# NeuralRevenant/semantic-query-engine

Measured on AMD Instinct MI355X. Metric: k-NN queries/sec (brute-force cosine top-10, 1024-d, 10M vectors), higher is better.
Workload: dtype i8; 1 GPU; flat cosine top-10, N=10000000 x 1024 fp32 (int8 collect scan (per-row-scaled int8 copy, sample-derived thresholds) + fp32 re-score of the candidates, exactness certified per query, bf16 collect pass for uncertified queries), batch=1024 queries/step, index row-sharded over 1 GPU(s); rows=10000000, dim=1024, batch=1024, k=10, parallelism=shard1, scan_mode=int8

## Files before the change

### semantic_query_engine_amd/csrc/exact.hip

```cpp
#include "kernels.h"

namespace sqe {

namespace {

struct RescoreArgs {
    const float* master;
    const float* qn;
    int K, B, k;
    const int* unc_ids;
    const int* unc_count;
    const float* collect_thr;
    uint64_t* keys;
    const int* key_cnt;
    float* cos_out;
    int64_t* id_out;
    int64_t id_base;
};

__global__ __launch_bounds__(256) void collect_rescore_kernel(RescoreArgs p) {
    __shared__ int hist[256];
    __shared__ int scratch[4];
    __shared__ uint64_t top[MAX_KP];
    const int ci = blockIdx.x;
// ... 90 lines not shown
            thr_out[ci] = collect_thr[q];
        }
        __syncthreads();
        if (tid == 0) {
            int t = 0;
            for (int w = 0; w < 16; ++w) t += wave_tot[w];
            base += t;
        }
        __syncthreads();
    }
    const int count = base;
    if (tid == 0) *unc_count = count;
    for (int i = count + tid; i < thr_cap; i += 1024) thr_out[i] = INFINITY;
    __syncthreads();
    const int vec_per_row = row_bytes / 16;
    for (int64_t e = tid; e < (int64_t)count * vec_per_row; e += 1024) {
        const int ci = (int)(e / vec_per_row), v = (int)(e - (int64_t)ci * vec_per_row);
        const uint4* src = reinterpret_cast<const uint4*>(reinterpret_cast<const char*>(qb) + (size_t)unc_ids[ci] * pitch_bytes);
        uint4* dst = reinterpret_cast<uint4*>(reinterpret_cast<char*>(qb_out) + (size_t)ci * pitch_bytes);
        dst[v] = src[v];
    }
}

}

int launch_compact_uncertified(const float* collect_thr, int B, const bf16_t* qb, int pitch_bytes, int row_bytes, int* unc_ids,
                               float* thr_out, int thr_cap, bf16_t* qb_out, int* unc_count, hipStream_t stream) {
    if (B <= 0) return SQE_OK;
    hipLaunchKernelGGL(compact_uncertified_kernel, dim3(1), dim3(1024), 0, stream, collect_thr, B, qb, pitch_bytes, row_bytes,
                       unc_ids, thr_out, thr_cap, qb_out, unc_count);
    SQE_HIP(hipGetLastError());
    return SQE_OK;
}

int launch_collect_rescore(const ExactArgs& a, hipStream_t stream) {
    if (a.B <= 0) return SQE_OK;
    if (a.K % 4 != 0) return fail(SQE_ERR_INVALID, "collect rescore: dim must be a multiple of 4");
    RescoreArgs p;
    p.master = a.master; p.qn = a.qn; p.K = a.K; p.B = a.B; p.k = a.k; p.collect_thr = a.collect_thr;
    p.unc_ids = a.unc_ids; p.unc_count = a.unc_count;
    p.keys = a.keys; p.key_cnt = a.key_cnt; p.cos_out = a.cos_out; p.id_out = a.id_out; p.id_base = a.id_base;
    hipLaunchKernelGGL(collect_rescore_kernel, dim3(a.B), dim3(256), 0, stream, p);
    SQE_HIP(hipGetLastError());
    return SQE_OK;
}

// ... 2 lines not shown
```

### semantic_query_engine_amd/csrc/internal.h

```cpp
#pragma once

#include <atomic>
#include <mutex>
#include <string>
#include <vector>

#include "kernels.h"

namespace sqe {

struct DevBuf {
    void* p = nullptr;
    size_t bytes = 0;
    DevBuf() = default;
    DevBuf(const DevBuf&) = delete;
    DevBuf& operator=(const DevBuf&) = delete;
    ~DevBuf() { release(); }
    void release() {
        if (p) (void)hipFree(p);
        p = nullptr;
        bytes = 0;
    }
    int ensure(size_t need) {
        if (need <= bytes) return SQE_OK;
// ... 144 lines not shown
    sqe::DevBuf dbg;
    sqe::DevBuf resid_max;
    sqe::DevBuf q_resid;
    sqe::DevBuf unc;
    sqe::DevBuf fb_keys, fb_cnt;
    sqe::DevBuf unc_ids, thr_c, qb_c;
    sqe::DevBuf stage_in, stage_out;
    int certify = 1;
    sqe::DevBuf i8db;
    sqe::DevBuf i8sxi;
    sqe::DevBuf i8resid_max;
    int64_t i8_cap_tiles = 0, i8_tile_stride = 0;
    int64_t i8_rows = 0;
    sqe::DevBuf q8t;
    sqe::DevBuf q8, q8sqi, q8resid, i8thr_int, i8thr_eff, i8cos_s, i8ids_s, i8stats, i8samp;
    int64_t i8_min_rows = 1000000;
    int i8_sample_step = 100;
    int i8_sample_m = 20;
    float i8_dx = 0.f;
    bool i8_dx_stale = true;
    bool i8_oom_logged = false;
    int i8_sample_int8 = 1;
    double i8_max_resid = 0.02;
    sqe::DevBuf i8ovf, i8ovf_cnt;
    double i8_anchor_margin = 0.25;
    int i8_key_budget = 6144;
    sqe_i8_launch_t i8_launch{};
    int last_B = 0;
    bool last_i8 = false;
    sqe::IvfState* ivf = nullptr;
    bool internal = false;
    sqe::GroupIndex* group = nullptr;
    std::atomic<int64_t> next_id{0};
    bool has_map = false;
    sqe::DevBuf idmap;
    sqe::FilterState* filter = nullptr;
    int64_t filter_gather_rows = 1 << 20;
    sqe::RangeState* range = nullptr;
    int64_t range_key_budget = 1 << 25;
    bool has_keys = false;
    sqe::DevBuf keys;
    sqe::CollapseState* collapse = nullptr;
    int collapse_depth = 0;
};

struct sqe_cache {
// ... 37 lines not shown
    bool locked;
    OpScope(sqe_ctx* c, OpOrder& ord, bool host_call, bool lock = true) : o(ord), locked(lock) {
        (void)hipSetDevice(c->device);
        if (locked) o.mu.lock();
        s = (host_call && !c->foreign.load()) ? o.own : c->stream.load();
        if (o.armed && o.last != s) (void)hipStreamWaitEvent(s, o.ev, 0);
    }
    ~OpScope() {
        (void)hipEventRecord(o.ev, s);
        o.last = s;
        o.armed = true;
        if (locked) o.mu.unlock();
    }
    OpScope(const OpScope&) = delete;
    OpScope& operator=(const OpScope&) = delete;
};

int index_create_impl(sqe_ctx* ctx, int dim, int kind, int nlist, bool internal, sqe_index** out);
int index_grow(sqe_index* idx, int64_t need_rows, hipStream_t s);
int index_add_impl(sqe_index* idx, const float* x_dev, int64_t n, int64_t x_stride, bool restore, hipStream_t s);
int index_update_impl(sqe_index* idx, const int64_t* rows_dev, const float* x_dev, int64_t n, hipStream_t s);
int index_search_impl(sqe_index* idx, const float* q_dev, int B, int k, int nprobe, float* cos_out_dev, int64_t* id_out_dev,
                      hipStream_t s, int pass_index = 0);

int ivf_create(sqe_index* base, IvfState** out);
void ivf_destroy(IvfState* st);
int ivf_rows_added(sqe_index* base, IvfState* st, hipStream_t s);
int ivf_rows_updated(sqe_index* base, IvfState* st, const int64_t* rows_dev, int64_t n, hipStream_t s);
int ivf_train(sqe_index* base, IvfState* st, const float* x_dev, int64_t n, int iters, uint64_t seed, hipStream_t s);
int ivf_search(sqe_index* base, IvfState* st, const float* q_dev, int B, int k, int nprobe, float* cos_out, int64_t* id_out,
               hipStream_t s);
int ivf_export(sqe_index* base, IvfState* st, float* centroids_host, int32_t* assign_host, hipStream_t s);
void ivf_invalidate(IvfState* st);
sqe_index* ivf_coarse(IvfState* st);
bool ivf_trained(IvfState* st);
int ivf_restore(sqe_index* base, IvfState* st, const float* centroids_dev, const int32_t* assign_dev, int64_t n, hipStream_t s);
void ivf_assignments(IvfState* st, int** assign, int64_t* n_assigned);
void ivf_rows_deleted(IvfState* st, int64_t n_assigned);

int64_t search_id_base(const sqe_index* idx);
int index_translate_ids(sqe_index* idx, int64_t* id_dev, int64_t count, hipStream_t s);
int index_resolve_ids(sqe_index* idx, const int64_t* ids_host, int64_t m, std::vector<int64_t>& pos, hipStream_t s, const char* what);
int index_delete_positions(sqe_index* idx, const std::vector<int64_t>& pos_sorted, hipStream_t s);
int index_ids_host(sqe_index* idx, std::vector<int64_t>& out, hipStream_t s);
int index_set_ids(sqe_index* idx, const int64_t* ids_host, int64_t next_id, hipStream_t s);
int launch_idmap_iota(int64_t* map, int64_t first_pos, int64_t first_id, int64_t n, hipStream_t s);
// ... 60 lines not shown
```

### semantic_query_engine_amd/csrc/search.hip

```cpp
#include <stdio.h>
#include <stdlib.h>
#include <string.h>

#include <algorithm>
#include <tuple>
#include <utility>

#include "internal.h"

namespace sqe {

__global__ void add_count_kernel(int* acc, const int* v) { *acc += *v; }

namespace {

int auto_kp(const sqe_index* idx, int k) {
    if (idx->rescore_k > 0) return std::min(MAX_KP, std::max(idx->rescore_k, k));
    if (idx->certify) return k <= 32 ? 64 : k <= 128 ? 128 : k;
    return std::min(MAX_KP, std::max(32, 4 * k));
}

struct Pass {
    sqe_index* idx;
    hipStream_t s;
    int64_t n_rows;
    int B, k, kp;
    ScanPlan plan;
    float* cos_out;
    int64_t* id_out;
    int pass_index;
    bool certify;
    int* unc_count;
    float* collect_thr;
    int step8, m8;
};

bool i8_stamps_wanted() {
    static const bool want_stamps = [] { const char* e = knob_env("SQE_I8_STAMPS"); return e && e[0] == '1'; }();
    return want_stamps;
}

bool scan_counters_wanted() {
    static const bool want = [] { const char* e = knob_env("SQE_DBG"); return e && (atoi(e) & 32); }();
    return want;
}

int arm_dbg(sqe_index* idx, hipStream_t s, unsigned long long** slot) {
    SQE_TRY(idx->dbg.ensure(8192));
    SQE_HIP(hipMemsetAsync(idx->dbg.p, 0, 8192, s));
    *slot = idx->dbg.as<unsigned long long>();
    return SQE_OK;
}

int report_i8_stamps(sqe_index* idx, hipStream_t s) {
    unsigned long long h[256];
    SQE_HIP(hipMemcpyAsync(h, idx->dbg.p, sizeof(h), hipMemcpyDeviceToHost, s));
    SQE_HIP(hipStreamSynchronize(s));
    int wall_khz = 0;
// ... 109 lines not shown
        idx->i8_tile_stride = stride;
    }
    if (!idx->i8resid_max.p) {
        SQE_TRY(idx->i8resid_max.ensure(16));
        SQE_HIP(hipMemsetAsync(idx->i8resid_max.p, 0, 16, s));
    }
    if (idx->i8_rows < n_rows) {
        StageTimer t(idx->ctx->prof, s, ST_ADD);
        SQE_TRY(launch_quantize_rows_i8(idx->master, nullptr, idx->i8_rows, n_rows - idx->i8_rows, n_rows, K, idx->i8db.as<int8_t>(), stride,
                                        idx->i8sxi.as<uint32_t>(), idx->i8resid_max.as<uint32_t>(), s));
        idx->i8_rows = n_rows;
        idx->i8_dx_stale = true;
    }
    if (idx->i8_dx_stale) {
        uint32_t bits = 0;
        SQE_HIP(hipMemcpyAsync(&bits, idx->i8resid_max.p, 4, hipMemcpyDeviceToHost, s));
        SQE_HIP(hipStreamSynchronize(s));
        memcpy(&idx->i8_dx, &bits, 4);
        idx->i8_dx_stale = false;
    }
    return SQE_OK;
}

int prepare_pass(Pass& p, const float* q_dev) {
    sqe_index* idx = p.idx;
    sqe_ctx* c = idx->ctx;
    const ScanPlan& plan = p.plan;
    hipStream_t s = p.s;
    const int K = idx->dim, B = p.B;
    SQE_TRY(idx->qn.ensure((size_t)B * K * 4));
    SQE_TRY(idx->qb.ensure((size_t)plan.b_pad * idx->pitch));
    SQE_TRY(idx->cand.ensure((size_t)plan.n_chunks * plan.b_pad * CAND_CAP * 8));
    SQE_TRY(idx->cand_cnt.ensure((size_t)plan.n_chunks * plan.b_pad * 4));
    const size_t gmax_bytes = (size_t)plan.b_pad * plan.ngroups * GMAX_COLS * 4;
    SQE_TRY(idx->gmax.ensure(gmax_bytes));
    static const bool no_collect = [] { const char* e = knob_env("SQE_NO_COLLECT"); return e && atoi(e) != 0; }();
    p.certify = idx->certify && p.n_rows > 0 && !no_collect;
    SQE_TRY(idx->q_resid.ensure((size_t)B * 4));
    if (p.certify) {
        SQE_TRY(idx->unc.ensure(16 + (size_t)plan.b_pad * 4));
        SQE_TRY(idx->fb_keys.ensure((size_t)B * EXACT_CAP * 8));
        SQE_TRY(idx->fb_cnt.ensure((size_t)B * 4));
        SQE_TRY(idx->unc_ids.ensure((size_t)B * 4));
        SQE_TRY(idx->thr_c.ensure((size_t)(plan.b_pad + 256) * 4));
        if ((size_t)(plan.b_pad + 256) * idx->pitch > idx->qb_c.bytes) {
            SQE_TRY(idx->qb_c.ensure((size_t)(plan.b_pad + 256) * idx->pitch));
            SQE_HIP(hipMemsetAsync(idx->qb_c.p, 0, idx->qb_c.bytes, s));
        }
    }
    {
        StageTimer t(c->prof, s, ST_PREP);
        if (plan.b_pad > B)
            SQE_HIP(hipMemsetAsync(idx->qb.as<char>() + (size_t)B * idx->pitch, 0, (size_t)(plan.b_pad - B) * idx->pitch, s));
        SQE_TRY(launch_normalize_rows(q_dev, B, K, K, idx->qn.as<float>(), idx->qb.as<bf16_t>(), idx->pitch / 2,
                                      idx->q_resid.as<float>(), nullptr, s));
        if (p.certify) {
            SQE_HIP(hipMemsetAsync(idx->unc.p, 0, 16, s));
            SQE_HIP(hipMemsetAsync(idx->fb_cnt.p, 0, (size_t)B * 4, s));
        }
        SQE_HIP(hipMemsetAsync(idx->gmax.p, 0, gmax_bytes, s));
    }
    p.unc_count = p.certify ? idx->unc.as<int>() : nullptr;
    p.collect_thr = p.certify ? reinterpret_cast<float*>(idx->unc.as<int>() + 4) : nullptr;
    return SQE_OK;
}

std::pair<int, int> sample_plan(int64_t n_rows, int step8, int m8) {
    const int64_t tiles = (n_rows + SCAN_BM - 1) / SCAN_BM;
    const int min_tiles = 2 * GMAX_COLS;
    if (tiles / step8 < min_tiles && tiles / min_tiles >= 1 && tiles / min_tiles < step8) {
        const int step_e = (int)std::max<int64_t>(std::max(1, (step8 * m8 + 63) / 64), tiles / min_tiles);
        const int m_e = std::min(64, std::max(m8, (step8 * m8 + step_e - 1) / step_e));
        step8 = step_e;
        m8 = m_e;
    }
    return {step8, m8};
}

int admit_i8(const Pass& p, bool* use) {
    sqe_index* idx = p.idx;
    const int K = idx->dim;
    *use = idx->scan_mode == SQE_SCAN_INT8_RESCORE && p.certify && K >= 256 && K % 128 == 0 && p.k <= p.m8 &&
           p.n_rows >= idx->i8_min_rows && p.n_rows >= (int64_t)p.step8 * SCAN_BM * 4;
    if (!*use) return SQE_OK;
    const int rc8 = ensure_i8_copy(idx, p.s);
    if (rc8 == SQE_ERR_OOM) {
// ... 2 lines not shown
        idx->scan_mode = SQE_SCAN_BF16_RESCORE;
        *use = false;
    } else {
        SQE_TRY(rc8);
        *use = idx->i8_dx <= (float)idx->i8_max_resid;
    }
    return SQE_OK;
}

ScanArgs bf16_scan_args(const Pass& p, const bf16_t* q) {
    sqe_index* idx = p.idx;
    ScanArgs a;
    a.db = idx->scan; a.q = q; a.n_rows = p.n_rows; a.K = idx->dim; a.B = p.B;
    a.db_pitch = idx->pitch; a.q_pitch = idx->pitch;
    a.cand = idx->cand.as<uint64_t>(); a.cand_cnt = idx->cand_cnt.as<int>(); a.gmax = idx->gmax.as<uint32_t>();
    return a;
}

int run_collect_fallback(const Pass& p) {
    sqe_index* idx = p.idx;
    sqe_ctx* c = idx->ctx;
    hipStream_t s = p.s;
    const int K = idx->dim, B = p.B;
    {
        StageTimer t(c->prof, s, ST_SELECT);
        SQE_TRY(launch_compact_uncertified(p.collect_thr, B, idx->qb.as<bf16_t>(), idx->pitch, K * 2, idx->unc_ids.as<int>(),
                                           idx->thr_c.as<float>(), p.plan.b_pad + 256, idx->qb_c.as<bf16_t>(), p.unc_count, s));
    }
    {
        StageTimer t(c->prof, s, ST_COLLECT);
        ScanArgs a = bf16_scan_args(p, idx->qb_c.as<bf16_t>());
        a.collect_thr = idx->thr_c.as<float>(); a.collect_keys = idx->fb_keys.as<uint64_t>(); a.collect_cnt = idx->fb_cnt.as<int>();
        a.unc_count = p.unc_count;
        const int bounds[5] = {0, 64, 256, 512, 1 << 30};
        for (int r = 0; r < 4 && bounds[r] < B; ++r) {
            const int hi = std::min(bounds[r + 1], B);
            const ScanPlan cp = make_scan_plan(p.n_rows, hi, p.kp, c->cu_count);
            a.collect_lo = bounds[r] + 1;
            a.collect_hi = r == 3 ? (1 << 30) : bounds[r + 1];
            SQE_TRY(launch_scan_collect(cp, a, s));
        }
    }
    {
        StageTimer t(c->prof, s, ST_SELECT);
        ExactArgs e;
        e.master = idx->master; e.qn = idx->qn.as<float>(); e.K = K; e.B = B; e.k = p.k;
        e.collect_thr = p.collect_thr; e.keys = idx->fb_keys.as<uint64_t>(); e.key_cnt = idx->fb_cnt.as<int>();
// ... 68 lines not shown
        ia.qblocks = plan.qblocks; ia.bn = plan.bn; ia.cand = idx->cand.as<uint64_t>(); ia.cand_cnt = idx->cand_cnt.as<int>();
        ia.ovf = idx->i8ovf.as<uint64_t>(); ia.ovf_cnt = idx->i8ovf_cnt.as<int>();
        if (i8_stamps_wanted()) SQE_TRY(arm_dbg(idx, s, &ia.stamps));
        static const int deep_max = [] { const char* e = knob_env("SQE_I8_DEEP_MAX"); return e ? atoi(e) : 1; }();
        if (plan.bn == 256 && plan.qblocks <= deep_max) SQE_TRY(launch_scan_i8_deep(ia, s));
        else SQE_TRY(launch_scan_i8(ia, s));
        if (i8_stamps_wanted()) SQE_TRY(report_i8_stamps(idx, s));
    }
    {
        StageTimer t(c->prof, s, ST_SELECT);
        I8SelectArgs sa;
        sa.cand = idx->cand.as<uint64_t>(); sa.cand_cnt = idx->cand_cnt.as<int>(); sa.n_chunks = plan.n_chunks; sa.b_pad = plan.b_pad;
        sa.master = idx->master; sa.qn = idx->qn.as<float>(); sa.K = K; sa.B = B; sa.k = p.k;
        sa.scan16 = idx->scan; sa.pitch16 = idx->pitch;
        sa.sxi = idx->i8sxi.as<uint32_t>(); sa.sqi = idx->q8sqi.as<uint32_t>();
        sa.q_resid8 = idx->q8resid.as<float>(); sa.db_resid8_max = idx->i8resid_max.as<uint32_t>();
        sa.q_resid16 = idx->q_resid.as<float>(); sa.db_resid16_max = idx->resid_max.as<uint32_t>();
        sa.thr_eff = idx->i8thr_eff.as<float>();
        sa.sample_cos = idx->i8cos_s.as<float>(); sa.sample_ids = idx->i8ids_s.as<int64_t>(); sa.sample_m = p.m8;
        sa.cos_out = p.cos_out; sa.id_out = p.id_out; sa.id_base = search_id_base(idx);
        sa.unc_count = p.unc_count; sa.collect_thr = p.collect_thr;
        sa.stats = idx->i8stats.as<unsigned long long>();
        sa.ovf = idx->i8ovf.as<uint64_t>(); sa.ovf_cnt = idx->i8ovf_cnt.as<int>();
        SQE_TRY(launch_select_i8(sa, s));
    }
    return SQE_OK;
}

int i8_first_pass(const Pass& p) {
    sqe_index* idx = p.idx;
    sqe_ctx* c = idx->ctx;
    const ScanPlan& plan = p.plan;
    hipStream_t s = p.s;
    const int K = idx->dim, B = p.B, step8 = p.step8, m8 = p.m8;
    const int q8_pitch = K + 128;
    const int b_pad_s = (B + 255) / 256 * 256;
    const int b_pad_q = std::max(plan.b_pad, b_pad_s);
    const int64_t full_tiles = p.n_rows / SCAN_BM;
    const int n_tiles_i8s = (int)(full_tiles / step8);
    const bool sample_i8 = idx->i8_sample_int8 != 0 && n_tiles_i8s >= 1;
    SQE_TRY(idx->q8.ensure((size_t)b_pad_q * q8_pitch));
    const size_t q8t_block = (size_t)256 * K;
    const size_t q8t_blocks = ((size_t)b_pad_q + 255) / 256;
    SQE_TRY(idx->q8t.ensure(q8t_blocks * q8t_block));
    SQE_TRY(idx->q8sqi.ensure((size_t)b_pad_q * 4));
    SQE_TRY(idx->q8resid.ensure((size_t)plan.b_pad * 4));
    SQE_TRY(idx->i8thr_int.ensure((size_t)plan.b_pad * 4));
    SQE_TRY(idx->i8thr_eff.ensure((size_t)plan.b_pad * 4));
    SQE_TRY(idx->i8cos_s.ensure((size_t)B * m8 * 4));
    SQE_TRY(idx->i8ids_s.ensure((size_t)B * m8 * 8));
    SQE_TRY(idx->i8stats.ensure(64));
    SQE_TRY(idx->i8ovf.ensure((size_t)plan.b_pad * I8_OVF_CAP * 8));
    SQE_TRY(idx->i8ovf_cnt.ensure((size_t)plan.b_pad * 4));
    {
        StageTimer t(c->prof, s, ST_PREP);
        SQE_HIP(hipMemsetAsync(idx->i8ovf_cnt.p, 0, (size_t)plan.b_pad * 4, s));
        if (b_pad_q > B)
            SQE_HIP(hipMemsetAsync(idx->q8.as<char>() + (size_t)B * q8_pitch, 0, (size_t)(b_pad_q - B) * q8_pitch, s));
        if (B % 256 != 0)
            SQE_HIP(hipMemsetAsync(idx->q8t.as<char>() + (size_t)(B / 256) * q8t_block, 0, (q8t_blocks - (size_t)(B / 256)) * q8t_block, s));
        SQE_TRY(launch_quantize_queries_i8(idx->qn.as<float>(), B, K, idx->q8.as<int8_t>(), q8_pitch, idx->q8t.as<int8_t>(),
                                           idx->q8sqi.as<uint32_t>(), idx->q8resid.as<float>(), s));
        SQE_HIP(hipMemsetAsync(idx->i8stats.p, 0, 64, s));
    }
    int chunks_s_used = 0;
    SQE_TRY(i8_threshold_pass(p, b_pad_s, n_tiles_i8s, sample_i8, &chunks_s_used));
    SQE_TRY(i8_scan_select(p, q8_pitch));
    SQE_TRY(run_collect_fallback(p));
    {
        sqe_i8_launch_t& L = idx->i8_launch;
        L.rows = p.n_rows; L.tile_stride = idx->i8_tile_stride; L.dim = K; L.B = B; L.b_pad = plan.b_pad; L.k = p.k;
        L.tile_rows = SCAN_BM; L.q_pitch = q8_pitch; L.query_block = plan.bn; L.n_chunks = plan.n_chunks; L.list_cap = CAND_CAP; L.pool_cap = I8_OVF_CAP;
        L.sample_int8 = sample_i8 ? 1 : 0; L.sample_step = step8; L.sample_tiles = n_tiles_i8s;
        L.sample_chunks = chunks_s_used;
        L.sample_b_pad = b_pad_s; L.sample_m = m8; L.uncertified = -1;
    }
    SQE_HIP(hipMemcpyAsync(c->i8_last.p, idx->i8stats.p, 32, hipMemcpyDeviceToDevice, s));
    c->i8_valid.store(true);
    return SQE_OK;
}

int bf16_first_pass(const Pass& p) {
    sqe_index* idx = p.idx;
    sqe_ctx* c = idx->ctx;
    const ScanPlan& plan = p.plan;
    hipStream_t s = p.s;
// ... 34 lines not shown
int search_positions(sqe_index* idx, const float* q_dev, int B, int k, int nprobe, float* cos_out_dev, int64_t* id_out_dev,
                     hipStream_t s, int pass_index) {
    sqe_ctx* c = idx->ctx;
    if (idx->ivf) {
        StageTimer t(c->prof, s, ST_SCAN);
        SQE_TRY(ivf_search(idx, idx->ivf, q_dev, B, k, nprobe > 0 ? nprobe : idx->nprobe, cos_out_dev, id_out_dev, s));
        c->search_calls++;
        return SQE_OK;
    }
    const int K = idx->dim;
    constexpr int MAX_PASS = 1024;
    if (B > MAX_PASS) {
        for (int off = 0; off < B; off += MAX_PASS) {
            const int m = std::min(MAX_PASS, B - off);
            SQE_TRY(search_positions(idx, q_dev + (size_t)off * K, m, k, nprobe, cos_out_dev + (size_t)off * k,
                                     id_out_dev + (size_t)off * k, s, off / MAX_PASS));
        }
        return SQE_OK;
    }
    Pass p{};
    p.idx = idx; p.s = s; p.n_rows = idx->n.load(); p.B = B; p.k = k; p.kp = auto_kp(idx, k);
    p.plan = make_scan_plan(p.n_rows, B, p.kp, c->cu_count, k);
    p.cos_out = cos_out_dev; p.id_out = id_out_dev; p.pass_index = pass_index;
    SQE_TRY(prepare_pass(p, q_dev));
    std::tie(p.step8, p.m8) = sample_plan(p.n_rows, idx->i8_sample_step, idx->i8_sample_m);
    bool use_i8 = false;
    SQE_TRY(admit_i8(p, &use_i8));
    if (use_i8) {
        SQE_TRY(i8_first_pass(p));
    } else {
        c->i8_valid.store(false);
        SQE_TRY(bf16_first_pass(p));
        if (p.certify) SQE_TRY(run_collect_fallback(p));
        SQE_TRY(report_scan_counters(p));
    }
    idx->last_B = B; idx->last_i8 = use_i8;
    book_search(p, use_i8 ? 1 : 2);
    return SQE_OK;
}

}

int index_search_positions(sqe_index* idx, const float* q_dev, int B, int k, int nprobe, float* cos_out_dev, int64_t* id_out_dev,
                           hipStream_t s) {
    return search_positions(idx, q_dev, B, k, nprobe, cos_out_dev, id_out_dev, s, 0);
}

int index_search_impl(sqe_index* idx, const float* q_dev, int B, int k, int nprobe, float* cos_out_dev, int64_t* id_out_dev,
                      hipStream_t s, int pass_index) {
    SQE_TRY(search_positions(idx, q_dev, B, k, nprobe, cos_out_dev, id_out_dev, s, pass_index));
// ... 5 lines not shown
```

### semantic_query_engine_amd/csrc/select_i8.hip

```cpp
#include "kernels.h"

namespace sqe {

namespace {

constexpr int KEY_CAP = 12288;
constexpr int RS_CAP = 4096;
constexpr int STAGE1 = 64;

struct SelArgs {
    I8SelectArgs a;
    float unit0;
};

__device__ __forceinline__ int key_score_i32(uint64_t key) { return (int)((uint32_t)(key >> 32) ^ 0x80000000u); }

__device__ __forceinline__ void rescore_range(const uint64_t* in, uint64_t* out, int lo, int hi, const float* master, const float* qrow, int K) {
    const int lane = threadIdx.x & 63, wave = threadIdx.x >> 6, nw = blockDim.x >> 6;
    const int nvec = K >> 2;
    const float4* qv = reinterpret_cast<const float4*>(qrow);
    for (int e = lo + wave * 2; e < hi; e += nw * 2) {
        const uint32_t r0 = key_row(in[e]);
        const bool two = e + 1 < hi;
        const uint32_t r1 = two ? key_row(in[e + 1]) : r0;
        const float4* a0 = reinterpret_cast<const float4*>(master + (size_t)r0 * K);
        const float4* a1 = reinterpret_cast<const float4*>(master + (size_t)r1 * K);
        float s0 = 0.f, s1 = 0.f;
        for (int v = lane; v < nvec; v += 64) {
            const float4 x0 = a0[v], x1 = a1[v], b = qv[v];
            s0 = fmaf(x0.x, b.x, s0); s0 = fmaf(x0.y, b.y, s0); s0 = fmaf(x0.z, b.z, s0); s0 = fmaf(x0.w, b.w, s0);
            s1 = fmaf(x1.x, b.x, s1); s1 = fmaf(x1.y, b.y, s1); s1 = fmaf(x1.z, b.z, s1); s1 = fmaf(x1.w, b.w, s1);
        }
        s0 = wave_sum(s0) + 0.0f;
        s1 = wave_sum(s1) + 0.0f;
        if (lane == 0) {
            out[e] = make_key(s0, r0);
            if (two) out[e + 1] = make_key(s1, r1);
        }
    }
}

__device__ __forceinline__ float dot8_bf16(const uint4 x, const float4 b0, const float4 b1, float s) {
    s = fmaf(__uint_as_float(x.x << 16), b0.x, s); s = fmaf(__uint_as_float(x.x & 0xffff0000u), b0.y, s);
    s = fmaf(__uint_as_float(x.y << 16), b0.z, s); s = fmaf(__uint_as_float(x.y & 0xffff0000u), b0.w, s);
    s = fmaf(__uint_as_float(x.z << 16), b1.x, s); s = fmaf(__uint_as_float(x.z & 0xffff0000u), b1.y, s);
    s = fmaf(__uint_as_float(x.w << 16), b1.z, s); s = fmaf(__uint_as_float(x.w & 0xffff0000u), b1.w, s);
    return s;
}
__device__ __forceinline__ void estimate_range_bf16(const uint64_t* in, uint64_t* out, int lo, int hi, const char* scan16, size_t pitch,
                                                    const float* qrow, int K) {
    constexpr int NR = 4;
    const int lane = threadIdx.x & 63, wave = threadIdx.x >> 6, nw = blockDim.x >> 6;
    const int nvec = K >> 3;
    const float4* qv = reinterpret_cast<const float4*>(qrow);
    for (int e = lo + wave * NR; e < hi; e += nw * NR) {
        uint32_t r[NR];
        const uint4* a[NR];
        float acc[NR];
#pragma unroll
        for (int i = 0; i < NR; ++i) {
            r[i] = key_row(in[min(e + i, hi - 1)]);
            a[i] = reinterpret_cast<const uint4*>(scan16 + (size_t)r[i] * pitch);
            acc[i] = 0.f;
        }
        for (int v = lane; v < nvec; v += 64) {
            uint4 x[NR];
#pragma unroll
            for (int i = 0; i < NR; ++i) x[i] = a[i][v];
            const float4 b0 = qv[2 * v], b1 = qv[2 * v + 1];
#pragma unroll
            for (int i = 0; i < NR; ++i) acc[i] = dot8_bf16(x[i], b0, b1, acc[i]);
        }
#pragma unroll
        for (int i = 0; i < NR; ++i) acc[i] = wave_sum(acc[i]) + 0.0f;
        if (lane == 0) {
#pragma unroll
            for (int i = 0; i < NR; ++i)
                if (e + i < hi) out[e + i] = make_key(acc[i], r[i]);
        }
    }
}

__device__ __forceinline__ void kth_largest(const uint64_t* v, int n, int k, uint64_t* out) {
    for (int i = threadIdx.x; i < n; i += blockDim.x) {
        const uint64_t me = v[i];
        int rank = 0;
        for (int j = 0; j < n; ++j) rank += v[j] > me ? 1 : 0;
        if (rank == k - 1) *out = me;
    }
}

constexpr int S1_TARGET = 64, S1_CAP = 256, NBIN = 1024;

__global__ __launch_bounds__(1024) void select_i8_kernel(SelArgs sa) {
    const I8SelectArgs& p = sa.a;
    __shared__ uint64_t keys[KEY_CAP];
    __shared__ uint64_t tk[RS_CAP];
    __shared__ int s_total, s_over, s_min, s_max, s_cutbin, s_n1, s_n2, s_n3, s_wtot[16];
    __shared__ uint64_t s_kth;
    const int q = blockIdx.x;
    const int tid = threadIdx.x, lane = tid & 63, wave = tid >> 6;
    if (tid == 0) {
        s_total = 0; s_over = 0; s_min = 0x7fffffff; s_max = (int)0x80000000; s_cutbin = 0; s_n1 = 0; s_n2 = 0; s_n3 = 0; s_kth = 0ull;
    }
    __syncthreads();
    for (int c = wave; c <= p.n_chunks; c += (int)(blockDim.x >> 6)) {
        const bool pool = c == p.n_chunks;
        int n = pool ? p.ovf_cnt[q] : min(p.cand_cnt[(size_t)c * p.b_pad + q], CAND_CAP);
        if (pool && n > I8_OVF_CAP) { n = I8_OVF_CAP; if (lane == 0) s_over = 1; }
        if (n <= 0) continue;
        int base = 0;
        if (lane == 0) base = atomicAdd(&s_total, n);
        base = __shfl(base, 0, 64);
        const uint64_t* list = pool ? p.ovf + (size_t)q * I8_OVF_CAP : p.cand + ((size_t)c * p.b_pad + q) * CAND_CAP;
        for (int i = lane; i < n; i += 64)
            if (base + i < KEY_CAP) keys[base + i] = list[i];
    }
    __syncthreads();
    int N = s_total;
    bool overflow = s_over != 0;
    if (N > KEY_CAP) { N = KEY_CAP; overflow = true; }
    {
        int lo = 0x7fffffff, hi = (int)0x80000000;
        for (int i = tid; i < N; i += blockDim.x) {
            const int sc = key_score_i32(keys[i]);
            lo = min(lo, sc); hi = max(hi, sc);
        }
#pragma unroll
        for (int off = 32; off > 0; off >>= 1) {
            lo = min(lo, __shfl_xor(lo, off, 64));
            hi = max(hi, __shfl_xor(hi, off, 64));
        }
        if (lane == 0 && lo <= hi) { atomicMin(&s_min, lo); atomicMax(&s_max, hi); }
    }
    int* hist = reinterpret_cast<int*>(tk);
    for (int i = tid; i < NBIN; i += blockDim.x) hist[i] = 0;
    __syncthreads();
    const long long smin = s_min, range = (long long)s_max - smin + 1;
    auto bin_of = [&](int sc) { return (int)((((long long)sc - smin) * NBIN) / range); };
    for (int i = tid; i < N; i += blockDim.x) atomicAdd(&hist[bin_of(key_score_i32(keys[i]))], 1);
    __syncthreads();
    {
// ... 8 lines not shown
        __syncthreads();
        int before = 0;
        for (int w = 0; w < wave; ++w) before += s_wtot[w];
        incl += before;
        if (incl >= S1_TARGET && incl - mine < S1_TARGET) s_cutbin = NBIN - 1 - tid;
    }
    __syncthreads();
    const int cutbin = s_cutbin;
    for (int i = tid; i < N; i += blockDim.x) {
        const uint64_t key = keys[i];
        if (bin_of(key_score_i32(key)) >= cutbin) {
            const int at = atomicAdd(&s_n1, 1);
            if (at < S1_CAP) {
                tk[at] = key;
                keys[i] = 0ull;
            }
        }
    }
    __syncthreads();
    const float* qrow = p.qn + (size_t)q * p.K;
    const char* scan16 = reinterpret_cast<const char*>(p.scan16);
    const float eps16r = scan_eps(0.f, __uint_as_float(*p.db_resid16_max), p.K);
    const int R1 = min(s_n1, S1_CAP);
    estimate_range_bf16(tk, tk, 0, R1, scan16, (size_t)p.pitch16, qrow, p.K);
    __syncthreads();
    if (R1 >= p.k) kth_largest(tk, R1, p.k, &s_kth);
    __syncthreads();
    const float eps8 = scan_eps(p.q_resid8[q], __uint_as_float(*p.db_resid8_max), p.K);
    const double unit = (double)sa.unit0 * (double)p.sqi[q];
    int thr2 = -0x7fffffff;
    if (R1 >= p.k) {
        const float t1 = key_score(s_kth) - eps16r;
        const double v = floor(((double)t1 - (double)eps8) / unit) - 1.0;
        thr2 = v < -2.0e9 ? -0x7fffffff : v > 2.0e9 ? 0x7fffffff : (int)v;
    }
    if (tid == 0) s_n2 = R1;
    __syncthreads();
    for (int i = tid; i < N; i += blockDim.x) {
        const uint64_t key = keys[i];
        if (key != 0ull && key_score_i32(key) >= thr2) {
            const int at = atomicAdd(&s_n2, 1);
            if (at < RS_CAP) tk[at] = key;
        }
    }
    __syncthreads();
    int R2 = s_n2;
    if (R2 > RS_CAP) { R2 = RS_CAP; overflow = true; }
    estimate_range_bf16(tk, tk, R1, R2, scan16, (size_t)p.pitch16, qrow, p.K);
    __syncthreads();
    uint64_t* fk = keys;
    int R3 = R2;
    if (R2 > p.k) {
        kth_largest(tk, R2, p.k, &s_kth);
        __syncthreads();
        const uint64_t cut_key = make_key(key_score(s_kth) - 2.0f * eps16r, 0xFFFFFFFFu);
        for (int i = tid; i < R2; i += blockDim.x) {
            const uint64_t key = tk[i];
            if (key >= cut_key) fk[atomicAdd(&s_n3, 1)] = key;
        }
        __syncthreads();
        R3 = s_n3;
    } else {
        for (int i = tid; i < R2; i += blockDim.x) fk[i] = tk[i];
        __syncthreads();
    }
    rescore_range(fk, fk, 0, R3, p.master, qrow, p.K);
    __syncthreads();
    const int m = min(R3, p.k);
    float* cos_out = p.cos_out + (size_t)q * p.k;
    int64_t* id_out = p.id_out + (size_t)q * p.k;
    const bool from_sample = m < p.k;
// ... 5 lines not shown
            id_out[i] = is[i] >= 0 ? is[i] + p.id_base : -1;
        }
    } else {
        for (int i = tid; i < R3; i += blockDim.x) {
            const uint64_t me = fk[i];
            int rank = 0;
            for (int j = 0; j < R3; ++j) rank += fk[j] > me ? 1 : 0;
            if (rank < p.k) {
                cos_out[rank] = key_score(me);
                id_out[rank] = (int64_t)key_row(me) + p.id_base;
                if (rank == p.k - 1) s_kth = me;
            }
        }
    }
    __syncthreads();
    if (tid == 0) {
        const float kth = m >= p.k ? key_score(s_kth) : -INFINITY;
        const bool certified = !overflow && m >= p.k && p.thr_eff[q] + eps8 < kth;
        float thr = INFINITY;
        if (!certified) {
            const float eps16 = scan_eps(p.q_resid16[q], __uint_as_float(*p.db_resid16_max), p.K);
            const float lb = fmaxf(kth, cs[p.k - 1]);
            thr = (lb > -INFINITY ? lb : -1.0f) - eps16;
            atomicAdd(p.unc_count, 1);
        }
        p.collect_thr[q] = thr;
        if (p.stats) {
            atomicAdd(&p.stats[0], (unsigned long long)N);
            atomicAdd(&p.stats[1], (unsigned long long)R3);
            if (overflow) atomicAdd(&p.stats[2], 1ull);
            if (!certified) atomicAdd(&p.stats[3], 1ull);
        }
    }
}

constexpr int SS_CAP = 4096;
constexpr int SS_TOP = 256;

__global__ __launch_bounds__(1024) void i8_sample_select_kernel(I8SampleSelectArgs p, float unit0) {
    __shared__ uint64_t vals[SS_CAP];
    __shared__ uint64_t top[SS_TOP];
    __shared__ uint64_t fk[64];
    __shared__ int hist[1024];
    __shared__ int s_min, s_max, s_cutbin, s_ntop, s_wtot[16];
    __shared__ uint64_t s_mth;
    const int q = blockIdx.x, tid = threadIdx.x, lane = tid & 63, wave = tid >> 6;
    const int N = min(p.n_chunks * 16, SS_CAP);
    if (tid == 0) { s_min = 0x7fffffff; s_max = (int)0x80000000; s_cutbin = 0; s_ntop = 0; s_mth = 0ull; }
    hist[tid] = 0;
    __syncthreads();
    const int2* cand = reinterpret_cast<const int2*>(p.cand);
    int lo = 0x7fffffff, hi = (int)0x80000000;
    for (int i = tid; i < N; i += 1024) {
        const int2 v = cand[((size_t)(i >> 4) * p.b_pad_s + q) * 16 + (i & 15)];
        const bool ok = v.y >= 0;
// ... 87 lines not shown
        int mine = 0;
        for (int i = tid; i < N; i += 1024) mine += (vals[i] != 0ull && key_score_i32(vals[i]) >= t) ? 1 : 0;
#pragma unroll
        for (int off = 32; off > 0; off >>= 1) mine += __shfl_xor(mine, off, 64);
        if (lane == 0 && mine) atomicAdd(&s_ntop, mine);
    }
    __syncthreads();
    if (tid == 0) {
        const double unit = (double)unit0 * (double)p.sqi[q];
        const bool too_many = p.key_budget > 0 && (long long)s_ntop * p.step > (long long)p.key_budget;
        const int t = too_many ? s_min : s_cutbin;
        p.thr_int[q] = t;
        p.thr_eff[q] = (float)((double)t * unit * (1.0 + 1e-6) + 1e-7);
    }
}

__global__ void i8_pad_thresholds_kernel(int B, int b_pad, int* __restrict__ thr_int, float* __restrict__ thr_eff) {
    const int q = B + blockIdx.x * blockDim.x + threadIdx.x;
    if (q < b_pad) { thr_int[q] = 0x7fffffff; thr_eff[q] = INFINITY; }
}

}

int launch_select_i8(const I8SelectArgs& a, hipStream_t stream) {
    if (a.B <= 0) return SQE_OK;
    if (a.k < 1 || a.k > STAGE1 || a.k > a.sample_m) return fail(SQE_ERR_INVALID, "int8 select: k must be in [1, min(64, sample depth)]");
    if (a.K % 8 != 0 || a.pitch16 % 16 != 0 || !a.scan16) return fail(SQE_ERR_INVALID, "int8 select: dim must be a multiple of 8, the bf16 copy 16-byte aligned rows");
    SelArgs sa;
    sa.a = a;
    const float s0 = i8_scale_unit(a.K);
    sa.unit0 = s0 * s0;
    hipLaunchKernelGGL(select_i8_kernel, dim3(a.B), dim3(1024), 0, stream, sa);
    SQE_HIP(hipGetLastError());
    return SQE_OK;
}

int launch_i8_sample_select(const I8SampleSelectArgs& a, hipStream_t stream) {
    if (a.B <= 0) return SQE_OK;
    if (a.m < 1 || a.m > 64 || a.k < 1 || a.k > a.m || a.K % 4 != 0 || a.n_chunks < 1)
        return fail(SQE_ERR_INVALID, "int8 sample select: 1 <= k <= m <= 64");
    const float s0 = i8_scale_unit(a.K);
    hipLaunchKernelGGL(i8_sample_select_kernel, dim3(a.B), dim3(1024), 0, stream, a, s0 * s0);
    if (a.b_pad > a.B)
        hipLaunchKernelGGL(i8_pad_thresholds_kernel, dim3((a.b_pad - a.B + 255) / 256), dim3(256), 0, stream, a.B, a.b_pad, a.thr_int, a.thr_eff);
    SQE_HIP(hipGetLastError());
    return SQE_OK;
}

}
```

Measured before the change: 111,600 queries/s.

## Split int8 select into small/large LDS variants, fuse compaction and batch resets

The int8 select kernel is templated into a small-LDS variant (fewer keys, higher occupancy) that runs first, plus the full-size variant that only processes queries flagged as too big for the small one. The select kernel now also writes the uncertified-query compaction (ids, thresholds, bf16 query copy) directly, which removes the separate compact kernel. Per-chunk candidate counts are gathered with a wave prefix scan instead of shared atomics. Several small memsets are merged into one multi-range reset kernel. The cost is two select launches and more code paths, with behaviour controlled by environment knobs.

```diff
diff --git a/semantic_query_engine_amd/csrc/exact.hip b/semantic_query_engine_amd/csrc/exact.hip
--- a/semantic_query_engine_amd/csrc/exact.hip
+++ b/semantic_query_engine_amd/csrc/exact.hip
@@ -1,4 +1,6 @@
-#include "kernels.h"
+#include <algorithm>
+
+#include "internal.h"
 
 namespace sqe {
 
@@ -136,6 +138,22 @@
     }
 }
 
+__global__ __launch_bounds__(256) void reset_pass_kernel(PassReset r) {
+    const PassReset::Range g = r.r[blockIdx.y];
+    for (uint32_t i = blockIdx.x * 256 + threadIdx.x; i < g.words; i += gridDim.x * 256) g.p[i] = g.value;
+}
+
+}
+
+int launch_reset_pass(const PassReset& r, hipStream_t stream) {
+    if (r.n <= 0) return SQE_OK;
+    if (r.n > PassReset::MAX) return fail(SQE_ERR_INVALID, "reset pass: too many ranges");
+    uint32_t most = 0;
+    for (int i = 0; i < r.n; ++i) most = std::max(most, r.r[i].words);
+    const int blocks = (int)std::min<uint32_t>(128u, (most + 1023u) / 1024u);
+    hipLaunchKernelGGL(reset_pass_kernel, dim3(std::max(blocks, 1), r.n), dim3(256), 0, stream, r);
+    SQE_HIP(hipGetLastError());
+    return SQE_OK;
 }
 
 int launch_compact_uncertified(const float* collect_thr, int B, const bf16_t* qb, int pitch_bytes, int row_bytes, int* unc_ids,
diff --git a/semantic_query_engine_amd/csrc/internal.h b/semantic_query_engine_amd/csrc/internal.h
--- a/semantic_query_engine_amd/csrc/internal.h
+++ b/semantic_query_engine_amd/csrc/internal.h
@@ -190,6 +190,7 @@
     bool i8_oom_logged = false;
     int i8_sample_int8 = 1;
     double i8_max_resid = 0.02;
+    sqe::DevBuf i8big;
     sqe::DevBuf i8ovf, i8ovf_cnt;
     double i8_anchor_margin = 0.25;
     int i8_key_budget = 6144;
@@ -273,6 +274,24 @@
 int index_update_impl(sqe_index* idx, const int64_t* rows_dev, const float* x_dev, int64_t n, hipStream_t s);
 int index_search_impl(sqe_index* idx, const float* q_dev, int B, int k, int nprobe, float* cos_out_dev, int64_t* id_out_dev,
                       hipStream_t s, int pass_index = 0);
+
+struct I8SelectCompact {
+    int* unc_ids = nullptr; float* thr_c = nullptr;
+    const char* qb = nullptr; char* qb_c = nullptr;
+    int pitch = 0, row_bytes = 0;
+};
+int launch_select_i8_sized(const I8SelectArgs& args, unsigned char* big, const I8SelectCompact& compact, hipStream_t stream);
+struct PassReset {
+    static constexpr int MAX = 10;
+    struct Range { uint32_t* p; uint32_t words, value; } r[MAX];
+    int n = 0;
+    void add(void* p, size_t bytes, uint32_t value = 0u) {
+        if (bytes == 0) return;
+        if (n < MAX) r[n] = {static_cast<uint32_t*>(p), (uint32_t)(bytes / 4), value};
+        ++n;
+    }
+};
+int launch_reset_pass(const PassReset& r, hipStream_t stream);
 
 int ivf_create(sqe_index* base, IvfState** out);
 void ivf_destroy(IvfState* st);
diff --git a/semantic_query_engine_amd/csrc/search.hip b/semantic_query_engine_amd/csrc/search.hip
--- a/semantic_query_engine_amd/csrc/search.hip
+++ b/semantic_query_engine_amd/csrc/search.hip
@@ -33,7 +33,28 @@
     int* unc_count;
     float* collect_thr;
     int step8, m8;
+    bool self_compact;
 };
+
+int select_parts() {
+    static const int parts = [] { const char* e = knob_env("SQE_SELECT_PARTS"); const int v = e ? atoi(e) : 7; return (v & 2) ? v : (v & ~4); }();
+    return parts;
+}
+
+int apply_resets(const PassReset& r, hipStream_t s) {
+    if (select_parts() & 2) return launch_reset_pass(r, s);
+    for (int i = 0; i < r.n && i < PassReset::MAX; ++i) SQE_HIP(hipMemsetD32Async(r.r[i].p, (int)r.r[i].value, r.r[i].words, s));
+    return SQE_OK;
+}
+
+void base_resets(const Pass& p, PassReset& r) {
+    sqe_index* idx = p.idx;
+    if (p.plan.b_pad > p.B) r.add(idx->qb.as<char>() + (size_t)p.B * idx->pitch, (size_t)(p.plan.b_pad - p.B) * idx->pitch);
+    if (p.certify) {
+        r.add(idx->unc.p, 16);
+        r.add(idx->fb_cnt.p, (size_t)p.B * 4);
+    }
+}
 
 bool i8_stamps_wanted() {
     static const bool want_stamps = [] { const char* e = knob_env("SQE_I8_STAMPS"); return e && e[0] == '1'; }();
@@ -189,9 +210,8 @@
     return SQE_OK;
 }
 
-int prepare_pass(Pass& p, const float* q_dev) {
-    sqe_index* idx = p.idx;
-    sqe_ctx* c = idx->ctx;
+int prepare_buffers(Pass& p) {
+    sqe_index* idx = p.idx;
     const ScanPlan& plan = p.plan;
     hipStream_t s = p.s;
     const int K = idx->dim, B = p.B;
@@ -215,20 +235,24 @@
             SQE_HIP(hipMemsetAsync(idx->qb_c.p, 0, idx->qb_c.bytes, s));
         }
     }
-    {
-        StageTimer t(c->prof, s, ST_PREP);
-        if (plan.b_pad > B)
-            SQE_HIP(hipMemsetAsync(idx->qb.as<char>() + (size_t)B * idx->pitch, 0, (size_t)(plan.b_pad - B) * idx->pitch, s));
-        SQE_TRY(launch_normalize_rows(q_dev, B, K, K, idx->qn.as<float>(), idx->qb.as<bf16_t>(), idx->pitch / 2,
-                                      idx->q_resid.as<float>(), nullptr, s));
-        if (p.certify) {
-            SQE_HIP(hipMemsetAsync(idx->unc.p, 0, 16, s));
-            SQE_HIP(hipMemsetAsync(idx->fb_cnt.p, 0, (size_t)B * 4, s));
-        }
-        SQE_HIP(hipMemsetAsync(idx->gmax.p, 0, gmax_bytes, s));
-    }
     p.unc_count = p.certify ? idx->unc.as<int>() : nullptr;
     p.collect_thr = p.certify ? reinterpret_cast<float*>(idx->unc.as<int>() + 4) : nullptr;
+    return SQE_OK;
+}
+
+int prepare_queries(const Pass& p, const float* q_dev, bool use_i8) {
+    sqe_index* idx = p.idx;
+    hipStream_t s = p.s;
+    const int K = idx->dim;
+    StageTimer t(idx->ctx->prof, s, ST_PREP);
+    SQE_TRY(launch_normalize_rows(q_dev, p.B, K, K, idx->qn.as<float>(), idx->qb.as<bf16_t>(), idx->pitch / 2,
+                                  idx->q_resid.as<float>(), nullptr, s));
+    if (!use_i8) {
+        PassReset r;
+        base_resets(p, r);
+        SQE_TRY(apply_resets(r, s));
+    }
+    SQE_HIP(hipMemsetAsync(idx->gmax.p, 0, (size_t)p.plan.b_pad * p.plan.ngroups * GMAX_COLS * 4, s));
     return SQE_OK;
 }
 
@@ -277,7 +301,7 @@
     sqe_ctx* c = idx->ctx;
     hipStream_t s = p.s;
     const int K = idx->dim, B = p.B;
-    {
+    if (!p.self_compact) {
         StageTimer t(c->prof, s, ST_SELECT);
         SQE_TRY(launch_compact_uncertified(p.collect_thr, B, idx->qb.as<bf16_t>(), idx->pitch, K * 2, idx->unc_ids.as<int>(),
                                            idx->thr_c.as<float>(), p.plan.b_pad + 256, idx->qb_c.as<bf16_t>(), p.unc_count, s));
@@ -392,7 +416,12 @@
         sa.unc_count = p.unc_count; sa.collect_thr = p.collect_thr;
         sa.stats = idx->i8stats.as<unsigned long long>();
         sa.ovf = idx->i8ovf.as<uint64_t>(); sa.ovf_cnt = idx->i8ovf_cnt.as<int>();
-        SQE_TRY(launch_select_i8(sa, s));
+        I8SelectCompact sc;
+        if (p.self_compact) {
+            sc.unc_ids = idx->unc_ids.as<int>(); sc.thr_c = idx->thr_c.as<float>();
+            sc.qb = idx->qb.as<char>(); sc.qb_c = idx->qb_c.as<char>(); sc.pitch = idx->pitch; sc.row_bytes = K * 2;
+        }
+        SQE_TRY(launch_select_i8_sized(sa, (select_parts() & 1) ? idx->i8big.as<unsigned char>() : nullptr, sc, s));
     }
     return SQE_OK;
 }
@@ -422,16 +451,20 @@
     SQE_TRY(idx->i8stats.ensure(64));
     SQE_TRY(idx->i8ovf.ensure((size_t)plan.b_pad * I8_OVF_CAP * 8));
     SQE_TRY(idx->i8ovf_cnt.ensure((size_t)plan.b_pad * 4));
+    SQE_TRY(idx->i8big.ensure((size_t)B));
     {
         StageTimer t(c->prof, s, ST_PREP);
-        SQE_HIP(hipMemsetAsync(idx->i8ovf_cnt.p, 0, (size_t)plan.b_pad * 4, s));
-        if (b_pad_q > B)
-            SQE_HIP(hipMemsetAsync(idx->q8.as<char>() + (size_t)B * q8_pitch, 0, (size_t)(b_pad_q - B) * q8_pitch, s));
+        PassReset r;
+        base_resets(p, r);
+        r.add(idx->i8ovf_cnt.p, (size_t)plan.b_pad * 4);
+        r.add(idx->i8stats.p, 64);
+        if (b_pad_q > B) r.add(idx->q8.as<char>() + (size_t)B * q8_pitch, (size_t)(b_pad_q - B) * q8_pitch);
         if (B % 256 != 0)
-            SQE_HIP(hipMemsetAsync(idx->q8t.as<char>() + (size_t)(B / 256) * q8t_block, 0, (q8t_blocks - (size_t)(B / 256)) * q8t_block, s));
+            r.add(idx->q8t.as<char>() + (size_t)(B / 256) * q8t_block, (q8t_blocks - (size_t)(B / 256)) * q8t_block);
+        if (p.self_compact) r.add(idx->thr_c.p, (size_t)(plan.b_pad + 256) * 4, 0x7f800000u);
+        SQE_TRY(apply_resets(r, s));
         SQE_TRY(launch_quantize_queries_i8(idx->qn.as<float>(), B, K, idx->q8.as<int8_t>(), q8_pitch, idx->q8t.as<int8_t>(),
                                            idx->q8sqi.as<uint32_t>(), idx->q8resid.as<float>(), s));
-        SQE_HIP(hipMemsetAsync(idx->i8stats.p, 0, 64, s));
     }
     int chunks_s_used = 0;
     SQE_TRY(i8_threshold_pass(p, b_pad_s, n_tiles_i8s, sample_i8, &chunks_s_used));
@@ -512,10 +545,12 @@
     p.idx = idx; p.s = s; p.n_rows = idx->n.load(); p.B = B; p.k = k; p.kp = auto_kp(idx, k);
     p.plan = make_scan_plan(p.n_rows, B, p.kp, c->cu_count, k);
     p.cos_out = cos_out_dev; p.id_out = id_out_dev; p.pass_index = pass_index;
-    SQE_TRY(prepare_pass(p, q_dev));
+    SQE_TRY(prepare_buffers(p));
     std::tie(p.step8, p.m8) = sample_plan(p.n_rows, idx->i8_sample_step, idx->i8_sample_m);
     bool use_i8 = false;
     SQE_TRY(admit_i8(p, &use_i8));
+    p.self_compact = use_i8 && (select_parts() & 4) != 0;
+    SQE_TRY(prepare_queries(p, q_dev, use_i8));
     if (use_i8) {
         SQE_TRY(i8_first_pass(p));
     } else {
diff --git a/semantic_query_engine_amd/csrc/select_i8.hip b/semantic_query_engine_amd/csrc/select_i8.hip
--- a/semantic_query_engine_amd/csrc/select_i8.hip
+++ b/semantic_query_engine_amd/csrc/select_i8.hip
@@ -1,4 +1,6 @@
-#include "kernels.h"
+#include <stdio.h>
+
+#include "internal.h"
 
 namespace sqe {
 
@@ -6,11 +8,15 @@
 
 constexpr int KEY_CAP = 12288;
 constexpr int RS_CAP = 4096;
+constexpr int KEY_CAP_S = 6144;
+constexpr int RS_CAP_S = 1024;
 constexpr int STAGE1 = 64;
 
 struct SelArgs {
     I8SelectArgs a;
     float unit0;
+    unsigned char* big;
+    I8SelectCompact c;
 };
 
 __device__ __forceinline__ int key_score_i32(uint64_t key) { return (int)((uint32_t)(key >> 32) ^ 0x80000000u); }
@@ -47,9 +53,9 @@
     s = fmaf(__uint_as_float(x.w << 16), b1.z, s); s = fmaf(__uint_as_float(x.w & 0xffff0000u), b1.w, s);
     return s;
 }
+template <int NR>
 __device__ __forceinline__ void estimate_range_bf16(const uint64_t* in, uint64_t* out, int lo, int hi, const char* scan16, size_t pitch,
                                                     const float* qrow, int K) {
-    constexpr int NR = 4;
     const int lane = threadIdx.x & 63, wave = threadIdx.x >> 6, nw = blockDim.x >> 6;
     const int nvec = K >> 3;
     const float4* qv = reinterpret_cast<const float4*>(qrow);
@@ -92,32 +98,53 @@
 
 constexpr int S1_TARGET = 64, S1_CAP = 256, NBIN = 1024;
 
-__global__ __launch_bounds__(1024) void select_i8_kernel(SelArgs sa) {
+template <int KEY_CAP, int RS_CAP, bool SMALL, int WAVES>
+__global__ __launch_bounds__(1024, WAVES) void select_i8_kernel(SelArgs sa) {
     const I8SelectArgs& p = sa.a;
     __shared__ uint64_t keys[KEY_CAP];
     __shared__ uint64_t tk[RS_CAP];
-    __shared__ int s_total, s_over, s_min, s_max, s_cutbin, s_n1, s_n2, s_n3, s_wtot[16];
+    __shared__ int s_over, s_min, s_max, s_cutbin, s_n1, s_n2, s_n3, s_slot, s_wtot[16];
     __shared__ uint64_t s_kth;
+    constexpr int EST_NR = SMALL ? 2 : 4;
+    static_assert(RS_CAP * 8 >= NBIN * 4 && RS_CAP >= S1_CAP, "tk holds the histogram and the stage-1 keys");
     const int q = blockIdx.x;
+    if (!SMALL && sa.big && !sa.big[q]) return;
     const int tid = threadIdx.x, lane = tid & 63, wave = tid >> 6;
     if (tid == 0) {
-        s_total = 0; s_over = 0; s_min = 0x7fffffff; s_max = (int)0x80000000; s_cutbin = 0; s_n1 = 0; s_n2 = 0; s_n3 = 0; s_kth = 0ull;
-    }
-    __syncthreads();
-    for (int c = wave; c <= p.n_chunks; c += (int)(blockDim.x >> 6)) {
-        const bool pool = c == p.n_chunks;
-        int n = pool ? p.ovf_cnt[q] : min(p.cand_cnt[(size_t)c * p.b_pad + q], CAND_CAP);
-        if (pool && n > I8_OVF_CAP) { n = I8_OVF_CAP; if (lane == 0) s_over = 1; }
-        if (n <= 0) continue;
-        int base = 0;
-        if (lane == 0) base = atomicAdd(&s_total, n);
-        base = __shfl(base, 0, 64);
-        const uint64_t* list = pool ? p.ovf + (size_t)q * I8_OVF_CAP : p.cand + ((size_t)c * p.b_pad + q) * CAND_CAP;
+        s_over = 0; s_min = 0x7fffffff; s_max = (int)0x80000000; s_cutbin = 0; s_n1 = 0; s_n2 = 0; s_n3 = 0; s_slot = -1; s_kth = 0ull;
+    }
+    const int c_mine = lane * 16 + wave;
+    int n_mine = 0;
+    if (c_mine < p.n_chunks) n_mine = max(0, min(p.cand_cnt[(size_t)c_mine * p.b_pad + q], CAND_CAP));
+    else if (c_mine == p.n_chunks) n_mine = max(0, p.ovf_cnt[q]);
+    bool pool_over = false;
+    if (c_mine == p.n_chunks && n_mine > I8_OVF_CAP) { n_mine = I8_OVF_CAP; pool_over = true; }
+    int base_mine = n_mine;
+#pragma unroll
+    for (int off = 1; off < 64; off <<= 1) {
+        const int o = __shfl_up(base_mine, off, 64);
+        if (lane >= off) base_mine += o;
+    }
+    __syncthreads();
+    if (lane == 63) s_wtot[wave] = base_mine;
+    if (pool_over) s_over = 1;
+    __syncthreads();
+    base_mine -= n_mine;
+    for (int w = 0; w < wave; ++w) base_mine += s_wtot[w];
+    int N = 0;
+    for (int w = 0; w < 16; ++w) N += s_wtot[w];
+    if (SMALL && N > KEY_CAP) {
+        if (tid == 0) sa.big[q] = 1;
+        return;
+    }
+    for (uint64_t m = __ballot(n_mine > 0); m; m &= m - 1) {
+        const int l = __ffsll((unsigned long long)m) - 1;
+        const int n = __shfl(n_mine, l, 64), base = __shfl(base_mine, l, 64), c = l * 16 + wave;
+        const uint64_t* list = c == p.n_chunks ? p.ovf + (size_t)q * I8_OVF_CAP : p.cand + ((size_t)c * p.b_pad + q) * CAND_CAP;
         for (int i = lane; i < n; i += 64)
             if (base + i < KEY_CAP) keys[base + i] = list[i];
     }
     __syncthreads();
-    int N = s_total;
     bool overflow = s_over != 0;
     if (N > KEY_CAP) { N = KEY_CAP; overflow = true; }
     {
@@ -172,7 +199,7 @@
     const char* scan16 = reinterpret_cast<const char*>(p.scan16);
     const float eps16r = scan_eps(0.f, __uint_as_float(*p.db_resid16_max), p.K);
     const int R1 = min(s_n1, S1_CAP);
-    estimate_range_bf16(tk, tk, 0, R1, scan16, (size_t)p.pitch16, qrow, p.K);
+    estimate_range_bf16<EST_NR>(tk, tk, 0, R1, scan16, (size_t)p.pitch16, qrow, p.K);
     __syncthreads();
     if (R1 >= p.k) kth_largest(tk, R1, p.k, &s_kth);
     __syncthreads();
@@ -195,8 +222,12 @@
     }
     __syncthreads();
     int R2 = s_n2;
+    if (SMALL && R2 > RS_CAP) {
+        if (tid == 0) sa.big[q] = 1;
+        return;
+    }
     if (R2 > RS_CAP) { R2 = RS_CAP; overflow = true; }
-    estimate_range_bf16(tk, tk, R1, R2, scan16, (size_t)p.pitch16, qrow, p.K);
+    estimate_range_bf16<EST_NR>(tk, tk, R1, R2, scan16, (size_t)p.pitch16, qrow, p.K);
     __syncthreads();
     uint64_t* fk = keys;
     int R3 = R2;
@@ -248,15 +279,27 @@
             const float eps16 = scan_eps(p.q_resid16[q], __uint_as_float(*p.db_resid16_max), p.K);
             const float lb = fmaxf(kth, cs[p.k - 1]);
             thr = (lb > -INFINITY ? lb : -1.0f) - eps16;
-            atomicAdd(p.unc_count, 1);
+            const int slot = atomicAdd(p.unc_count, 1);
+            if (sa.c.unc_ids) {
+                sa.c.unc_ids[slot] = q;
+                sa.c.thr_c[slot] = thr;
+                s_slot = slot;
+            }
         }
         p.collect_thr[q] = thr;
+        if (SMALL) sa.big[q] = 0;
         if (p.stats) {
             atomicAdd(&p.stats[0], (unsigned long long)N);
             atomicAdd(&p.stats[1], (unsigned long long)R3);
             if (overflow) atomicAdd(&p.stats[2], 1ull);
             if (!certified) atomicAdd(&p.stats[3], 1ull);
         }
+    }
+    __syncthreads();
+    if (s_slot >= 0) {
+        const uint4* src = reinterpret_cast<const uint4*>(sa.c.qb + (size_t)q * sa.c.pitch);
+        uint4* dst = reinterpret_cast<uint4*>(sa.c.qb_c + (size_t)s_slot * sa.c.pitch);
+        for (int v = tid; v < sa.c.row_bytes / 16; v += 1024) dst[v] = src[v];
     }
 }
 
@@ -390,18 +433,37 @@
 
 }
 
-int launch_select_i8(const I8SelectArgs& a, hipStream_t stream) {
+int launch_select_i8_sized(const I8SelectArgs& a, unsigned char* big, const I8SelectCompact& compact, hipStream_t stream) {
     if (a.B <= 0) return SQE_OK;
+    if (a.n_chunks >= 1024) return fail(SQE_ERR_INVALID, "int8 select: at most 1,023 chunk lists per query");
+    if (compact.unc_ids && (!compact.thr_c || !compact.qb || !compact.qb_c || compact.pitch % 16 != 0 || compact.row_bytes % 16 != 0))
+        return fail(SQE_ERR_INVALID, "int8 select: the dense batch needs its thresholds and 16-byte aligned bf16 rows");
     if (a.k < 1 || a.k > STAGE1 || a.k > a.sample_m) return fail(SQE_ERR_INVALID, "int8 select: k must be in [1, min(64, sample depth)]");
     if (a.K % 8 != 0 || a.pitch16 % 16 != 0 || !a.scan16) return fail(SQE_ERR_INVALID, "int8 select: dim must be a multiple of 8, the bf16 copy 16-byte aligned rows");
     SelArgs sa;
     sa.a = a;
     const float s0 = i8_scale_unit(a.K);
     sa.unit0 = s0 * s0;
-    hipLaunchKernelGGL(select_i8_kernel, dim3(a.B), dim3(1024), 0, stream, sa);
+    sa.big = big;
+    sa.c = compact;
+    static const bool reported = [] {
+        const char* e = knob_env("SQE_SELECT_REPORT");
+        if (!e || e[0] != '1') return false;
+        int ns = 0, nl = 0;
+        (void)hipOccupancyMaxActiveBlocksPerMultiprocessor(&ns, select_i8_kernel<KEY_CAP_S, RS_CAP_S, true, 8>, 1024, 0);
+        (void)hipOccupancyMaxActiveBlocksPerMultiprocessor(&nl, select_i8_kernel<KEY_CAP, RS_CAP, false, 4>, 1024, 0);
+        fprintf(stderr, "[sqe select_i8] resident workgroups per CU: small (%d keys, %d estimates) %d, large (%d, %d) %d\n",
+                KEY_CAP_S, RS_CAP_S, ns, KEY_CAP, RS_CAP, nl);
+        return true;
+    }();
+    (void)reported;
+    if (big) hipLaunchKernelGGL((select_i8_kernel<KEY_CAP_S, RS_CAP_S, true, 8>), dim3(a.B), dim3(1024), 0, stream, sa);
+    hipLaunchKernelGGL((select_i8_kernel<KEY_CAP, RS_CAP, false, 4>), dim3(a.B), dim3(1024), 0, stream, sa);
     SQE_HIP(hipGetLastError());
     return SQE_OK;
 }
+
+int launch_select_i8(const I8SelectArgs& a, hipStream_t stream) { return launch_select_i8_sized(a, nullptr, I8SelectCompact{}, stream); }
 
 int launch_i8_sample_select(const I8SampleSelectArgs& a, hipStream_t stream) {
     if (a.B <= 0) return SQE_OK;
```

Result: no change. 111,400 queries/s (median of 2 runs) (-0.2%).
